# hobincar/reconstruction-network-for-video-captioning

Hardware: AMD Instinct MI355X
Metric: captions/sec (train step) MSVD bs=100 28x1536 feats (higher is better)
Workload: dtype bf16; 1 GPU; decoder + global reconstructor train step (fwd+bwd+clip+Adam), B=100 per GPU, F=28, D=R=1536, V=4188, E=468, H=512, A=128, T=31, dropout 0.5, LSTM cells; global_batch=100, parallelism=dp1, hipgraph=True, deferred_reconstructor_update=True, grad_allreduce=False

## Files before the change

### reconstruction-network-for-video-captioning_amd/csrc/abi_step.inc

```

int recnet_set_deferred_reconstructor_update(recnet_handle* h, int32_t on, void* stream) {
  REQUIRE_WS(h);
  FLUSH_PENDING(h, stream);
  h->defer_rec = on ? (on == 2 ? 2 : 1) : 0;
  LAUNCH_OK();
  return RECNET_OK;
}
int recnet_flush(recnet_handle* h, void* stream) {
  REQUIRE_WS(h);
  int r = flush_pending(h, (hipStream_t)stream, 1); if (r) return r;
  LAUNCH_OK();
  return RECNET_OK;
}
int recnet_set_dp_overlap(recnet_handle* h, int32_t on) {
  if (!h) return fail(RECNET_EINVAL, "null handle");
  h->dp_overlap = on ? 1 : 0;
  return RECNET_OK;
}
int recnet_join_side(recnet_handle* h, void* stream) {
  REQUIRE_WS(h);
  if (h->side_open && h->s2) { hipEventRecord(h->ev[14], h->s2); hipStreamWaitEvent((hipStream_t)stream, h->ev[14], 0); }
  h->side_open = 0;
  LAUNCH_OK();
  return RECNET_OK;
}
int recnet_abort_step(recnet_handle* h) {
  if (!h) return fail(RECNET_EINVAL, "null handle");
  h->dp_overlap = 0; h->side_open = 0; h->in_fused = 0; h->defer_now = 0; h->defer_err = 0;
  h->total_late = 0; h->side_tail_open = 0; h->rec_wait_pending = 0; h->rec_norm_late = 0; h->rec_loss_late = 0; h->rec_loss_defer = 0; h->prezeroed = 0; h->norms_hoisted = 0; h->hoist_pending = 0;
  h->hoist_fork_recorded = 0; h->side_fork_recorded = 0; h->encmean_hoisted = 0; h->ctx_done = 0; h->side_pending = 0;
  h->join_pending = 0; h->join_recorded = 0; h->deferred_done = 0; h->deferred_early = 0; h->early_opt_done = 0;
  h->xcat_done = 0; h->mp_done = 0; h->dhr_done = 0; h->dout_ready = 0; h->gg_slots = 0; h->gemm_single_group = 0;
  h->img_defer_now = 0; h->s3_late = 0;
  h->gws_cur = h->gws;
  return RECNET_OK;
}
int recnet_mark_pending(recnet_handle* h) {
  if (!h) return fail(RECNET_EINVAL, "null handle");
  if (h->defer_rec) { h->maybe_pending = 1; h->images_maybe_stale = 1; }
  return RECNET_OK;
}

int recnet_forward_decoder(recnet_handle* h, const float* enc, const int64_t* targets, int32_t T,
                           const float* step_weight, int32_t train, uint32_t seed, float* hiddens_out,
                           recnet_scalars* scalars, void* stream) {
  REQUIRE_WS(h);
  if (!h->dec_bound) return fail(RECNET_ESTATE, "decoder not bound");
  if (!enc || !targets || !step_weight) return fail(RECNET_EINVAL, "null argument");
  if (check_T(h, T)) return fail(RECNET_EINVAL, "T out of range");
  hipStream_t st = (hipStream_t)stream;
  hipLaunchKernelGGL(set_u32_kernel, dim3(1), dim3(1), 0, st, h->ctrl, seed);
  int r = fwd_decoder(h, enc, targets, T, step_weight, train, hiddens_out, st); if (r) return r;
  if (scalars) hipLaunchKernelGGL(export_scalars_kernel, dim3(1), dim3(1), 0, st, h->scal, scalars);
  LAUNCH_OK();
  return RECNET_OK;
}
// ... 150 lines not shown
    hipLaunchKernelGGL(mean_over_f_kernel, dim3(ew_blocks((size_t)h->B * h->D)), dim3(256), 0, sn, h->hoist_enc, h->B, h->F, h->D, h->encmean);
    h->encmean_hoisted = 1;
  }
  if (sn != st) hipEventRecord(h->ev[5], sd);
}

static void side_after_decoder_fwd(recnet_handle* h, hipStream_t st) {
  hipStream_t sd = h->overlap ? h->s2 : st;
  const bool par = sd != st;
  h->side_pending = 0;
  if (par) {
    if (h->side_fork_recorded) {
      hipStreamWaitEvent(sd, h->ev[0], 0);
      if (h->kind == RECNET_REC_GLOBAL && h->persist_rec) wait_chain(h, 2, sd);
    } else fork_to(h, 0, st, sd);
    h->side_fork_recorded = 0; h->gws_cur = h->gws2;
  }
  h->join_pending = par; h->join_recorded = 0; h->side_tail_open = 0;
  if (par && h->kind != RECNET_REC_NONE) h->gg_slots = 2 * (h->ncu > 192 ? h->ncu - 192 : 32);
  int r = dec_fwd_loss(h, h->side_targets, h->side_T, h->side_stepw, 1, sd);
  if (!r) r = dec_bwd_out(h, 1.0f, sd);
  h->gg_slots = 0;
  if (!r && par && h->side_phase != 2) { dec_ctx_rows(h, h->side_enc, 0, h->side_T, sd); h->ctx_done = 1; }
  if (h->side_tail_open) hipEventRecord(h->ev[18], sd);
  h->gws_cur = h->gws;
  h->side_err = r;
}

static int fwd_bwd_impl(recnet_handle* h, const float* enc, const int64_t* targets, int T, const float* stepw, hipStream_t st,
                        int phase, int early_opt) {
  const bool rec = h->kind != RECNET_REC_NONE;
  hipStream_t sd = h->overlap ? h->s2 : st;
  const bool par = sd != st;
  int r;
  bool s3_join = false;
  const float* dh = rec ? h->dHsrec : nullptr;
  h->early_opt_done = 0;
  if (phase != 2) h->free_fwd = 0;
  if (phase != 2) h->ctx_done = 0;
  const bool defer_static = h->defer_rec && (h->kind == RECNET_REC_GLOBAL || (h->defer_rec == 2 && h->kind == RECNET_REC_LOCAL)) && phase == 0 && early_opt >= 0 && par && h->s3 &&
                            (h->defer_rec != 2 || h->split_ok);
  const bool defer = defer_static && (h->defer_rec != 2 || T >= 2);
  if (!defer && h->defer_rec && phase != 2) {
    if (defer_static) { const int fr = flush_pending(h, st, 1); if (fr) return fr; }
    else if (h->maybe_pending) { const int fr = flush_pending(h, st, 0); if (fr) return fr; }
  }
// ... 110 lines not shown

int recnet_train_step_fwd_bwd(recnet_handle* h, const float* enc, const int64_t* targets, int32_t T,
                              const float* step_weight, uint32_t seed, recnet_scalars* scalars, void* stream) {
  REQUIRE_WS(h);
  FLUSH_PENDING(h, stream);
  if (!h->dec_bound || (h->kind != RECNET_REC_NONE && !h->rec_bound)) return fail(RECNET_ESTATE, "models not bound");
  if (!h->dGd.out_weight || (h->kind != RECNET_REC_NONE && !h->rG.out_weight)) return fail(RECNET_ESTATE, "gradients not bound");
  if (!enc || !targets || !step_weight) return fail(RECNET_EINVAL, "null argument");
  if (check_T(h, T)) return fail(RECNET_EINVAL, "T out of range");
  hipStream_t st = (hipStream_t)stream;
  hipLaunchKernelGGL(set_u32_kernel, dim3(1), dim3(1), 0, st, h->ctrl, seed);
  int r = fwd_bwd(h, enc, targets, T, step_weight, st); if (r) return r;
  if (scalars) hipLaunchKernelGGL(export_scalars_kernel, dim3(1), dim3(1), 0, st, h->scal, scalars);
  h->fwd_dec_done = 0;
  LAUNCH_OK();
  return RECNET_OK;
}

static void step_fail_cleanup(recnet_handle* h, hipStream_t st) {
  if (h->s3_late && h->s3) join_from(h, 11, st, h->s3);
  recnet_abort_step(h);
  if (h->defer_rec) { h->maybe_pending = 1; h->images_maybe_stale = 1; }
}
static int check_step_args(recnet_handle* h, const float* enc, const int64_t* targets, int T, const float* step_weight) {
  if (!h->dec_bound || (h->kind != RECNET_REC_NONE && !h->rec_bound)) return fail(RECNET_ESTATE, "models not bound");
  if (!h->dGd.out_weight || (h->kind != RECNET_REC_NONE && !h->rG.out_weight)) return fail(RECNET_ESTATE, "gradients not bound");
  if (!enc || !targets || !step_weight) return fail(RECNET_EINVAL, "null argument");
  if (check_T(h, T)) return fail(RECNET_EINVAL, "T out of range");
  return RECNET_OK;
}

int recnet_train_step(recnet_handle* h, const float* enc, const int64_t* targets, int32_t T,
                      const float* step_weight, uint32_t seed, int32_t step, recnet_scalars* scalars, void* stream) {
  REQUIRE_WS(h);
  if (!h->defer_rec) { const int fr_ = flush_pending(h, (hipStream_t)stream); if (fr_) return fr_; }
  int r = check_step_args(h, enc, targets, T, step_weight); if (r) return r;
  if (step < 1) return fail(RECNET_EINVAL, "step must be >= 1");
  hipStream_t st = (hipStream_t)stream;
  const int flags = RECNET_OPT_REG | RECNET_OPT_CLIP;
  hipLaunchKernelGGL(set_u32_kernel, dim3(1), dim3(1), 0, st, h->ctrl, seed);
  hipLaunchKernelGGL(set_step_kernel, dim3(1), dim3(1), 0, st, (int32_t*)(h->ctrl + 1), step);
  h->in_fused = 1;
  r = fwd_bwd(h, enc, targets, T, step_weight, st, 0, flags); if (r) { h->in_fused = 0; return r; }
  r = optimizer_step(h, flags, st, h->early_opt_done ? 0 : -1); h->in_fused = 0;
  if (r) { step_fail_cleanup(h, st); return r; }
  if (h->s3_late) { join_from(h, 11, st, h->s3); h->s3_late = 0; }
  h->img_defer_now = 0;
  if (scalars) hipLaunchKernelGGL(export_scalars_kernel, dim3(1), dim3(1), 0, st, h->scal, scalars);
  h->fwd_dec_done = 0;
  LAUNCH_OK();
  return RECNET_OK;
}

int recnet_train_step_dev(recnet_handle* h, const float* enc, const int64_t* targets, int32_t T, const float* step_weight,
                          uint32_t seed_base, int32_t flags, recnet_scalars* scalars, void* stream) {
  REQUIRE_WS(h);
  if (!h->defer_rec) { const int fr_ = flush_pending(h, (hipStream_t)stream); if (fr_) return fr_; }
  int r = check_step_args(h, enc, targets, T, step_weight); if (r) return r;
  hipStream_t st = (hipStream_t)stream;
  hipLaunchKernelGGL(advance_step_kernel, dim3(1), dim3(1), 0, st, (int32_t*)(h->ctrl + 1), h->ctrl, seed_base);
  h->in_fused = 1;
  r = fwd_bwd(h, enc, targets, T, step_weight, st, 0, flags); if (r) { h->in_fused = 0; return r; }
  r = optimizer_step(h, flags, st, h->early_opt_done ? 0 : -1); h->in_fused = 0;
  if (r) { step_fail_cleanup(h, st); return r; }
  if (h->s3_late) { join_from(h, 11, st, h->s3); h->s3_late = 0; }
  h->img_defer_now = 0;
  if (scalars) hipLaunchKernelGGL(export_scalars_kernel, dim3(1), dim3(1), 0, st, h->scal, scalars);
  h->fwd_dec_done = 0;
  LAUNCH_OK();
  return RECNET_OK;
}

int recnet_set_step(recnet_handle* h, int32_t step, void* stream) {
  REQUIRE_WS(h);
  hipLaunchKernelGGL(set_u32_kernel, dim3(1), dim3(1), 0, (hipStream_t)stream, h->ctrl + 1, (uint32_t)step);
  LAUNCH_OK();
  return RECNET_OK;
}

int recnet_train_step_fwd_bwd_dev(recnet_handle* h, const float* enc, const int64_t* targets, int32_t T,
                                  const float* step_weight, uint32_t seed_base, recnet_scalars* scalars, void* stream) {
  REQUIRE_WS(h);
  FLUSH_PENDING(h, stream);
  if (!h->dec_bound || (h->kind != RECNET_REC_NONE && !h->rec_bound)) return fail(RECNET_ESTATE, "models not bound");
  if (!h->dGd.out_weight || (h->kind != RECNET_REC_NONE && !h->rG.out_weight)) return fail(RECNET_ESTATE, "gradients not bound");
  if (!enc || !targets || !step_weight) return fail(RECNET_EINVAL, "null argument");
// ... 41 lines not shown
```

### reconstruction-network-for-video-captioning_amd/csrc/api.hip

```cpp
#include <hip/hip_runtime.h>
#include <math.h>
#include <stdio.h>
#include <stdlib.h>
#include <ctype.h>
#include <string.h>
#include <algorithm>
#include <string>
#include <vector>

#include "../../include/recnet_hip.h"
#include "kernels.hpp"
#include "rec_chain.hpp"
#include "dec_chain.hpp"
#include "loc_chain.hpp"
#include "loc_big.hpp"

static thread_local std::string g_err;
static int fail(int code, const std::string& m) { g_err = m; return code; }
#define HIPCHK(x) do { hipError_t e_ = (x); if (e_ != hipSuccess) return fail(RECNET_EHIP, std::string(#x) + ": " + hipGetErrorString(e_)); } while (0)
#define LAUNCH_OK() do { hipError_t e_ = hipGetLastError(); if (e_ != hipSuccess) return fail(RECNET_EHIP, std::string(__func__) + ": " + hipGetErrorString(e_)); } while (0)

static inline int cdiv(long a, long b) { return (int)((a + b - 1) / b); }
static inline int ew_blocks(size_t n) { size_t b = (n + 255) / 256; return (int)(b > 4096 ? 4096 : (b < 1 ? 1 : b)); }

struct OptGroup {
  std::vector<TensorDesc> tab;
  std::vector<int2> chunks;
  TensorDesc* d_tab = nullptr; int2* d_chunks = nullptr; PackDesc* d_pack = nullptr;
  std::vector<PackDesc> pack;
  float* d_partial = nullptr; float* d_pnorm = nullptr; float* d_gnorm = nullptr;
  int ntens = 0, nchunks = 0;
  bool bound = false;
};

static inline int pad8(int n) { return (n + 7) & ~7; }
#define RN_REC_T_WHH(h) ((h)->kind == RECNET_REC_LOCAL ? 5 : 1)
#define RN_GCNT_WORDS 16384
#define RN_MAX_ROW_GROUPS 4

struct recnet_handle {
  recnet_config c;
  int B, F, D, E, H, A, V, R, RA, Tm, kind, prec, cml;
  int dgru = 0, rgru = 0;
  int lp;
  int ldD, ldE, ldH, ldV, ldA, ld4H, ldWS, ldR, ld4R, ldRA, ldHR, ldRA4, ld2H;
  char* ws = nullptr; size_t ws_bytes = 0; size_t need = 0;
  uint32_t* ctrl;
  uint32_t* gbar;
  float* scal;
  float *slab2 = nullptr;
  float *bsum4 = nullptr, *bsum4r = nullptr;
  int prezeroed = 0;
  float *bsum_d, *Uv, *Xe, *Hs, *Cs, *acts, *Wh, *att, *logits, *rowloss, *slab, *gws, *dHs, *dHsrec, *dc_carry, *dUv,
      *dwacc, *demb, *stepw, *msep;
  void *enc_lp, *emb_lp, *Hs_lp, *P, *dlog_lp, *dGx, *ctx_lp, *dUv_lp, *dWhs;
  void *U_w, *Wc_w, *We_w, *Wcomb, *Wo_w;
  void* WcombT = nullptr;
  int ldKW = 0, use_wcomb_t = 0;
  float *bsum_r, *mp, *Xg, *Hr, *Cr, *acts_r, *hrmean, *outm, *encmean, *dhrmean, *dmpd, *dmp, *dcr_carry;
// ... 31 lines not shown
  int rec_norm_late = 0;
  int side_tail_open = 0;
  int total_late = 0;
  int split_ok = 0;
  int rec_wait_pending = 0;
  int defer_rec = 0, defer_now = 0, defer_err = 0, maybe_pending = 0, def_rows = 0, defer_flags = 3; hipStream_t s3 = nullptr; float* gws3 = nullptr;
  int mp_done = 0;
  int ncu = 0;
  int ctx_done = 0;
  int hoist_pending = 0, hoist_par = 0, encmean_hoisted = 0; const float* hoist_enc = nullptr;
  int xcat_done = 0;
  float* dc_G2 = nullptr; void* dc_pan2 = nullptr;
  void *Xcat_g, *Hr_lp, *hrmean_lp, *dout_lp, *dGr, *Xcat_r, *dUd_lp, *dWhr, *dWhrs, *Wr4_w;
  void *Wih_f, *Whh_w, *Wor_w, *Ur_w, *Wr_w, *Wihh_w;
  int persist_rec = 0;
  float *sr_logits, *sr_scores, *sr_h[2], *sr_c[2], *sr_hn, *sr_cn, *sr_cum[2], *sr_vals;
  int64_t *sr_tok[2], *sr_hist[2]; int32_t *sr_eos[2], *sr_idx;
  int64_t* in_tok = nullptr;
  int free_fwd = 0;
  size_t gws_floats, slab_floats;
  float* gws2 = nullptr; float* gws_cur = nullptr;
  unsigned* gcnt = nullptr;
  int gg_site = 0;
  struct RnSw { int wait_chain = 1, mse_epi = 1, adam_epi = 1, dec_lw = 1, dec_xcat = 1, rec_epi = 2, rec_wide = 1, persist_ms = 0, gemm_group = 1; } sw;
  int gg_slots = 0;
  int gemm_single_group = 0;
  hipStream_t s2 = nullptr; hipEvent_t ev[24] = {}; int overlap = 1;
  recnet_decoder_tensors dP{}, dGd{}, dM{}, dV{}, dVm{};
  recnet_reconstructor_tensors rP{}, rG{}, rM{}, rV{}, rVm{};
  bool dec_bound = false, rec_bound = false;
  OptGroup og[2];
  int T_last = 0, train_last = 0, fwd_dec_done = 0, fwd_rec_done = 0, rec_bwd_done = 0, early_opt_done = 0, norms_hoisted = 0, join_pending = 0;
  int prof_on = 0; std::vector<hipEvent_t> prof_ev; size_t prof_used = 0;
};

static size_t carve(recnet_handle* h, char* base) {
  size_t off = 0;
  auto take = [&](size_t nfloats) -> float* {
    float* p = base ? (float*)(base + off) : nullptr;
    off += ((nfloats * 4 + 255) / 256) * 256;
    return p;
  };
  auto takev = [&](size_t n) -> void* { return (void*)take(n); };
  const size_t B = h->B, F = h->F, D = h->D, E = h->E, H = h->H, A = h->A, V = h->V, R = h->R, RA = h->RA, Tm = h->Tm;
  h->ldD = pad8(h->D); h->ldE = pad8(h->E); h->ldH = pad8(h->H); h->ldV = pad8(h->V); h->ldA = pad8(h->A);
  h->ld4H = pad8(4 * h->H); h->ldWS = pad8(4 * h->H + RN_FCH * h->A);
  h->ldR = pad8(h->R); h->ld4R = pad8(4 * h->R); h->ldRA = pad8(h->RA); h->ldHR = pad8(h->H + h->R);
// ... 101 lines not shown
      if (h->lc_steps) h->Wst = takev((R / 16) * 4 * (size_t)(h->lc_steps - h->lc_sr) * 4 * 512 / 2 + 64);
    }
    h->lc_pang = takev(F * rc_pan_elems((int)(4 * R)) / 2 + 64);
    h->lc_panw = takev(F * rc_pan_elems((int)RA) / 2 + 64);
    h->lc_dx = take(F * 4 * B * H);
    h->WihhT = takev((H + R) * (size_t)h->ld4R);
    if (R > 2048 && R % 128 == 0 && B <= 64 * 2 * RN_MAX_ROW_GROUPS) {
      const int steps = (int)R / 128;
      h->lb_steps = steps; h->lb_sr = LB_SR(steps); h->lb_ncb = (int)(H + R) / 64;
      h->lb_part = take(F * 4 * 64 * (H + R));
      h->lb_dxm = take(F * B * H); h->lb_dbeta = take(F * B * Tm);
      h->WstT = takev((size_t)h->lb_ncb * 4 * 4 * (size_t)(steps - h->lb_sr) * 4 * 512 / 2 + 64);
    }
  }
  for (int g = 0; g < 2; ++g) {
    OptGroup& o = h->og[g];
    size_t nparams = g == 0 ? (V * E + A * H + A * D + 2 * A + 4 * H * (E + D) + 4 * H * H + 8 * H + V * H + V)
                            : (RA * R + RA * H + 2 * RA + 4 * R * 2 * H + 4 * R * R + 8 * R + R * R + R);
    size_t maxch = nparams / RN_CHUNK + 16;
    o.d_tab = (TensorDesc*)take(16 * sizeof(TensorDesc) / 4);
    o.d_pack = (PackDesc*)take(16 * sizeof(PackDesc) / 4);
    o.d_chunks = (int2*)take(maxch * 2);
    o.d_partial = take(maxch);
    o.d_pnorm = take(16);
    o.d_gnorm = take(16);
  }
  return off;
}

static DropDesc mkdrop(const recnet_handle* h, uint32_t site, float p, int train) {
  DropDesc d;
  d.seed = h->ctrl; d.site = site;
  d.thr = train ? rn_drop_thr(p) : 0u;
  d.inv_keep = (p < 1.f) ? 1.0f / (1.0f - p) : 0.f;
  d.Bg = h->c.global_batch_size; d.boff = h->c.batch_offset;
  return d;
}

extern "C" {

int recnet_abi_version(void) { return RECNET_ABI_VERSION; }
const char* recnet_last_error(void) { return g_err.c_str(); }

static std::vector<std::string> env_list(const char* var) {
  std::vector<std::string> out;
  const char* e = getenv(var);
// ... 13 lines not shown
int recnet_create(const recnet_config* cfg, recnet_handle** out) {
  if (!cfg || !out) return fail(RECNET_EINVAL, "null argument");
  const recnet_config& c = *cfg;
  if (c.batch_size <= 0 || c.encoder_output_len <= 0 || c.encoder_output_size <= 0 || c.embedding_size <= 0 ||
      c.decoder_hidden_size <= 0 || c.decoder_attn_size <= 0 || c.n_vocabs <= 3 || c.caption_max_len <= 0)
    return fail(RECNET_EINVAL, "non-positive dimension");
  if (c.reconstructor_type < 0 || c.reconstructor_type > 2) return fail(RECNET_EINVAL, "unknown reconstructor_type");
  if (c.precision != RECNET_PREC_F32 && c.precision != RECNET_PREC_BF16) return fail(RECNET_EINVAL, "unknown precision");
  if (c.decoder_attn_normalize != RECNET_ATTN_NONE && c.decoder_attn_normalize != RECNET_ATTN_SOFTMAX)
    return fail(RECNET_EINVAL, "unknown decoder_attn_normalize (0 = none, 1 = softmax)");
  if (c.decoder_cell < 0 || c.decoder_cell > 1 || c.reconstructor_cell < 0 || c.reconstructor_cell > 1)
    return fail(RECNET_EINVAL, "unknown recurrent cell (0 = LSTM, 1 = GRU)");
  if (c.reconstructor_type != RECNET_REC_NONE && c.reconstructor_hidden_size <= 0)
    return fail(RECNET_EINVAL, "reconstructor_hidden_size");
  if (c.reconstructor_type == RECNET_REC_LOCAL && c.reconstructor_hidden_size != c.encoder_output_size)
    return fail(RECNET_EINVAL, "local reconstructor requires reconstructor_hidden_size == encoder_output_size (train.py:128)");
  if (c.reconstructor_type == RECNET_REC_GLOBAL && c.reconstructor_hidden_size != c.encoder_output_size)
    return fail(RECNET_EINVAL, "global reconstructor requires reconstructor_hidden_size == encoder_output_size (train.py:101)");
  if (c.reconstructor_type == RECNET_REC_LOCAL && c.reconstructor_attn_size <= 0)
    return fail(RECNET_EINVAL, "reconstructor_attn_size");
  const std::vector<std::string> per_step = env_list("RN_PER_STEP"), alts = env_list("RN_ALT");
  const std::vector<std::string> per_step_names = {"dec", "dec_bwd", "rec", "rec_bwd", "loc", "loc_bwd", "loc_big", "all"};
  const std::vector<std::string> alt_names = {"dec_wh_in_phase_a", "dec_no_xcat", "rec_epilogue_0", "rec_epilogue_1", "rec_bwd_narrow",
                                              "rec_row_parts_1", "rec_row_parts_2", "loc_no_hybrid", "loc_xsplit_never", "loc_xsplit_always"};
  for (const std::string& t : per_step) if (!has(per_step_names, t)) return fail(RECNET_EINVAL, "RN_PER_STEP: unknown name '" + t + "'");
  for (const std::string& t : alts) if (!has(alt_names, t)) return fail(RECNET_EINVAL, "RN_ALT: unknown name '" + t + "'");
  auto alt = [&](const char* name) { return has(alts, name); };
  auto chain_on = [&](const char* name) { return !has(per_step, name) && !has(per_step, "all"); };
  recnet_handle* h = new recnet_handle();
  h->c = c;
  if (h->c.global_batch_size <= 0) h->c.global_batch_size = c.batch_size;
  h->B = c.batch_size; h->F = c.encoder_output_len; h->D = c.encoder_output_size; h->E = c.embedding_size;
  h->H = c.decoder_hidden_size; h->A = c.decoder_attn_size; h->V = c.n_vocabs;
  h->R = c.reconstructor_type ? c.reconstructor_hidden_size : 0;
  h->RA = c.reconstructor_type == RECNET_REC_LOCAL ? c.reconstructor_attn_size : 0;
  h->cml = c.caption_max_len; h->Tm = c.caption_max_len + 1;
  h->kind = c.reconstructor_type; h->prec = c.precision; h->lp = c.precision == RECNET_PREC_BF16;
  h->gemm_single_group = 0;
  {
    auto env = [](const char* n, int dflt) { const char* e = getenv(n); return e ? atoi(e) : dflt; };
    h->sw.wait_chain = env("RN_WAIT_CHAIN", 1); h->sw.mse_epi = env("RN_MSE_EPILOGUE", 1); h->sw.adam_epi = env("RN_ADAM_EPILOGUE", 1);
    h->sw.gemm_group = env("RN_GEMM_GROUP", 1);
    h->sw.dec_lw = !alt("dec_wh_in_phase_a");
    h->sw.dec_xcat = !alt("dec_no_xcat"); h->sw.rec_epi = alt("rec_epilogue_0") ? 0 : (alt("rec_epilogue_1") ? 1 : 2); h->sw.rec_wide = !alt("rec_bwd_narrow");
    h->sw.persist_ms = alt("rec_row_parts_1") ? 1 : (alt("rec_row_parts_2") ? 2 : 0);
  }
  h->dgru = c.decoder_cell == RECNET_CELL_GRU; h->rgru = c.reconstructor_type != RECNET_REC_NONE && c.reconstructor_cell == RECNET_CELL_GRU;
  {
    const char* eg = getenv("RN_ROW_GROUPS");
    int ng = (h->B + RC_PAN_ROWS - 1) / RC_PAN_ROWS;
    if (eg && atoi(eg) == 0 && ng > 1) ng = 0;
    h->bgrp = ng >= 1 && ng <= RN_MAX_ROW_GROUPS ? (h->B + ng - 1) / ng : h->B;
  }
  const int Bg = h->bgrp;
  {
    int dev = 0, ncu = 0;
    hipGetDevice(&dev);
    hipDeviceGetAttribute(&ncu, hipDeviceAttributeMultiprocessorCount, dev);
    h->ncu = ncu;
    h->persist_rec = chain_on("rec") && h->lp && h->kind == RECNET_REC_GLOBAL && Bg <= RC_PAN_ROWS && h->Tm <= 60 &&
                     (h->R & 7) == 0 && h->R <= 2048 && h->R / 8 <= ncu;
    const int N = 4 * h->H + h->A, NA = N / 16;
    h->persist_dec = chain_on("dec") && h->lp && h->Tm <= 60 && (h->H & 7) == 0 && h->H <= 512 && h->F <= 32 + DC_XF && h->A <= 128 &&
                     (N & 15) == 0 && Bg <= RC_PAN_ROWS && (NA > Bg ? NA : Bg) + 1 <= ncu;
    h->persist_rec_bwd = chain_on("rec_bwd") && h->persist_rec && (h->R & 15) == 0;
  }
  h->bgrp_loc = h->bgrp;
  {
// ... 252 lines not shown
```

### reconstruction-network-for-video-captioning_amd/csrc/host_reconstructor.inc

```
static void lstm_pw(recnet_handle* h, int Hd, int S, int slab_ld, const float* X, int x_ld, const float* b1, const float* b2,
                    const float* c_prev, float* h_out, void* h_lp, int hlp_ld, void* h_lp2, int hlp2_ld, float* c_out,
                    float* acts, hipStream_t st) {
  LstmPwArgs p;
  p.B = h->B; p.Hd = Hd; p.S = S; p.gru = h->rgru; p.slab = h->slab; p.slab_stride = (size_t)h->B * slab_ld; p.slab_ld = slab_ld;
  p.X = X; p.x_ld = x_ld; p.b1 = b1; p.b2 = b2; p.c_prev = c_prev; p.h_out = h_out; p.h_ld = Hd;
  p.h_lp = h_lp; p.hlp_ld = hlp_ld; p.hlp_pad_from = Hd; p.h_lp2 = h_lp2; p.hlp2_ld = hlp2_ld; p.c_out = c_out; p.acts = acts;
  auto al16 = [](const void* q) { return (((uintptr_t)q) & 15) == 0; };
  const bool vec = (Hd & 3) == 0 && (slab_ld & 3) == 0 && (x_ld & 3) == 0 && (hlp_ld & 3) == 0 && (hlp2_ld & 3) == 0 &&
                   al16(p.slab) && al16(X) && al16(b1) && al16(b2) && al16(c_prev) && al16(h_out) && al16(c_out) && al16(acts) &&
                   (((uintptr_t)h_lp) & 7) == 0 && (((uintptr_t)h_lp2) & 7) == 0;
  if (vec) LAUNCH_AT(h, lstm_pw_vec_kernel, dim3(cdiv((long)h->B * (Hd >> 2), 256)), dim3(256), 0, st, p);
  else LAUNCH_AT(h, lstm_pw_kernel, dim3(cdiv((long)h->B * Hd, 256)), dim3(256), 0, st, p);
}
static void mean_over_t(recnet_handle* h, const float* X, int T, int Cn, float scale, float* out, void* out_lp, int ld_lp, hipStream_t st) {
  const size_t n = (size_t)h->B * (out_lp ? ld_lp : Cn);
  if (h->lp) hipLaunchKernelGGL(mean_over_t_kernel<bf16_t>, dim3(ew_blocks(n)), dim3(256), 0, st, X, T, h->B, Cn, scale, out, (bf16_t*)out_lp, ld_lp);
  else hipLaunchKernelGGL(mean_over_t_kernel<float>, dim3(ew_blocks(n)), dim3(256), 0, st, X, T, h->B, Cn, scale, out, (float*)out_lp, ld_lp);
}

template <typename K, typename Args>
static void rc_launch(recnet_handle* h, int site, K kern, dim3 grid, size_t smem, hipStream_t st, const Args& a) {
  if (smem > 64 * 1024) hipFuncSetAttribute(reinterpret_cast<const void*>(kern), hipFuncAttributeMaxDynamicSharedMemorySize, (int)smem);
  hipEvent_t e1 = nullptr;
  if (h->prof_on == site) {
// ... 573 lines not shown
    }
    e.ad_pnorm = o.d_pnorm + ti;
  };
  if (!h->rgru) add(0, 4 * R, 0, dG1);
  else { add(0, 2 * R, 0, dG1); add((size_t)2 * R, R, (size_t)3 * R, at_off(h, (void*)dG1, (size_t)3 * R)); }
  h->gg_site = 3;
  if (!gg_run(h, g, s, &sh)) return false;
  if (local) { refresh_wst(h, s); refresh_wihh_t(h, s, 2); }
  return true;
}
static int optimizer_step(recnet_handle* h, int flags, hipStream_t st, int only_group, int deferred, int step_off, unsigned skip_mask) {
  RN_RANGE("recnet: norms + clip + Adam (train.py:270-273)");
  for (int g = 0; g < 2; ++g) {
    OptGroup& o = h->og[g];
    if (!o.bound) continue;
    if (only_group >= 0 && g != only_group) continue;
    if (g == 0 && (flags & RECNET_OPT_SKIP_DECODER)) continue;
    if (g == 1 && ((flags & RECNET_OPT_SKIP_RECONSTRUCTOR) || h->kind == RECNET_REC_NONE)) continue;
    if (!o.tab[0].m || !o.tab[0].g) return fail(RECNET_ESTATE, "gradients / Adam state not bound");
    AdamHyper hp = adam_hyper(h, g, flags);
    const float coef = hp.reg_coef;
    const float* clip = nullptr;
    if (g == 0 && (flags & RECNET_OPT_CLIP) && h->c.gradient_clip > 0.f) {
      hipLaunchKernelGGL(sumsq_chunk_kernel, dim3(o.nchunks), dim3(256), 0, st, o.d_tab, o.d_chunks, 1, o.d_pnorm, coef, o.d_partial);
      if (o.ntens <= 16) {
        hipLaunchKernelGGL(norm_all_kernel, dim3(1), dim3(256), 0, st, o.d_tab, o.d_partial, o.ntens, o.d_gnorm, h->c.gradient_clip, h->scal + 7, h->scal + 8, (float*)nullptr);
      } else {
        hipLaunchKernelGGL(tensor_norm_kernel, dim3(o.ntens), dim3(256), 0, st, o.d_tab, o.d_partial, o.d_gnorm);
        hipLaunchKernelGGL(norm_finalize_kernel, dim3(1), dim3(64), 0, st, o.d_gnorm, o.ntens, h->c.gradient_clip, h->scal + 7, h->scal + 8, (float*)nullptr);
      }
      clip = h->scal + 8;
    }
    hipLaunchKernelGGL(adam_chunk_kernel, dim3(o.nchunks), dim3(256), 0, st, o.d_tab, o.d_chunks, hp, o.d_pnorm, clip,
                       (const int32_t*)(h->ctrl + 1), (const PackDesc*)o.d_pack, h->lp, (const float*)(h->scal + 15),
                       deferred ? (const uint32_t*)(h->ctrl + 2) : (const uint32_t*)nullptr, step_off, g == 1 ? skip_mask : 0u);
    if (g == 0) refresh_wcomb_t(h, st);
    if (g == 1) rec_images_after_update(h, st, (skip_mask >> RN_REC_T_WHH(h)) & 1u);
  }
  return RECNET_OK;
}
```

### reconstruction-network-for-video-captioning_amd/csrc/loc_chain.hpp

```cpp
#pragma once
#include "common.hpp"
#include "rec_chain.hpp"

struct LocChainArgs {
  int F, T, B, R, H, A, gru;
  int Bs;
  int NU, NG, MS, NC;
  int relay;
  const bf16_t* W; int ldw;
  const bf16_t* Wr; int ldwr;
  const bf16_t* Wst;
  const float* bias;
  const float* Hs; const float* Ud;
  const float* ab; const float* w;
  float* Hr; float* Cr; float* acts;
  bf16_t* Hlp; int ld_hlp;
  bf16_t* Xcat; int ld_xcat;
  float* beta; float* Whr;
  bf16_t* PanH; bf16_t* PanX;
  _Float16* Pw;
  unsigned* bar; unsigned* epoch; float* poison;
  DropDesc dd;
  unsigned long long* ts;
};
// ... 32 lines not shown
  if (threadIdx.x < 64) {
    const unsigned* r = rel + (blockIdx.x & 7) * 32;
    unsigned spin = 0;
    while ((int)(__hip_atomic_load(r, __ATOMIC_RELAXED, __HIP_MEMORY_SCOPE_AGENT) - target) < 0) { if (rc_give_up(bar, spin)) break; }
    if (RC_ACQUIRE_INV) __builtin_amdgcn_fence(__ATOMIC_ACQUIRE, "agent");
  }
  __syncthreads();
}
__device__ __forceinline__ void lc_wait_or_relay(bool me, unsigned* rel, const unsigned* flags, int n, unsigned target, unsigned* bar) {
  if (!me) { lc_wait(rel, target, bar); return; }
  if (threadIdx.x < 64) {
    unsigned spin = 0;
    lc_poll(flags, n, target, bar, spin);
    lc_release(rel, target);
    if (RC_ACQUIRE_INV) __builtin_amdgcn_fence(__ATOMIC_ACQUIRE, "agent");
  }
  __syncthreads();
}
__device__ __forceinline__ void lc_arrive(unsigned* flag, unsigned v) {
  if (threadIdx.x == 0) __hip_atomic_store(flag, v, __ATOMIC_RELAXED, __HIP_MEMORY_SCOPE_AGENT);
}
__device__ __forceinline__ void lc_store16f(float* dst, f32x4 v) { rc_store16f(dst, v); }
__device__ __forceinline__ void lc_store16(bf16_t* dst, const bf16_t* src) { rc_store16(dst, src); }
#define LC_GLOBAL __attribute__((address_space(1)))
typedef const LC_GLOBAL bf16x8* lc_gbf16x8;
typedef const LC_GLOBAL f32x4* lc_gf32x4;
typedef const LC_GLOBAL float* lc_gf32;
template <typename T> __device__ __forceinline__ const LC_GLOBAL T* lc_launder_v(const T* ptr) { asm volatile("" : "+v"(ptr)); return (const LC_GLOBAL T*)ptr; }
template <typename T> __device__ __forceinline__ const LC_GLOBAL T* lc_launder_s(const T* ptr) { asm volatile("" : "+s"(ptr)); return (const LC_GLOBAL T*)ptr; }
typedef short lc_s4 __attribute__((ext_vector_type(4)));
typedef _Float16 lc_h4 __attribute__((ext_vector_type(4)));

template <int STEPS, int PF, int RB, int SR = STEPS, int NQ = 32>
__global__ __launch_bounds__(256) void loc_chain_kernel(const LocChainArgs p) {
  constexpr int CG = 4, UW = 16, ROWS = RB * 16, NP = STEPS / 2, KG = UW / 8, SX = 4, NPR = SR / 2;
  static_assert(SR % 2 == 0 && SR <= STEPS && SR >= 2 * PF, "resident k-steps: whole pairs, at least the prefetch distance");
  extern __shared__ __attribute__((aligned(16))) float lc_smem[];
  const int tid = threadIdx.x, lane = tid & 63, wave = __builtin_amdgcn_readfirstlane(tid >> 6);
  const int wg = blockIdx.x, R = p.R, B = p.B, Bs = p.Bs, H = p.H, A = p.A, F = p.F, T = p.T;
  const unsigned ep = rc_epoch_read(p.epoch), fb = ep << 7;
  unsigned* relU = p.bar + 256; unsigned* relC = p.bar + 256 + 16;
  const size_t pan_h = rc_pan_elems(R), pan_x = rc_pan_elems(H);

  if (p.relay && wg == p.NU + p.NC) {
    if (tid < 64) {
      unsigned spin = 0;
// ... 169 lines not shown
  }
  constexpr int CPT = (ROWS * UW + 255) / 256;
  static_assert(CPT == 4 || CPT == 2, "RB = 4 or 2");
#define LCU_CELL(c) (((tid / UW) * CPT + (c)) * UW + tid % UW)
  float xb[CPT][4], cpv[CPT];
  bool mine[CPT];
#pragma unroll
  for (int c = 0; c < CPT; ++c) {
    const int cell = LCU_CELL(c), rg = r0 + cell / UW;
    mine[c] = cell < ROWS * UW && rg >= own_lo && rg < own_lo + own && rg < B;
    cpv[c] = 0.f;
#pragma unroll
    for (int q = 0; q < 4; ++q) xb[c][q] = p.bias[q * R + u0 + cell % UW];
  }
  const int lane_off = ((lane >> 4) * RC_PAN_ROWS + r0 + (lane & 15)) * 8;
  f32x4 acc[RB][CG];
#pragma unroll
  for (int i = 0; i < RB; ++i)
#pragma unroll
    for (int g = 0; g < CG; ++g) acc[i][g] = f32x4{0.f, 0.f, 0.f, 0.f};
  const int it_j = tid / own, it_rg = own_lo + tid % own;
  const bool it_on = tid < KG * own && it_rg < B && it_rg - r0 < ROWS;
  const bf16_t* it_src = hl + (it_on ? it_rg - r0 : 0) * UW + (it_on ? it_j : 0) * 8;

  for (int s = 0; s < F; ++s) {
    lc_wait(relC, fb + (unsigned)(s + 1), p.bar);
    if (wg == 0) LC_TS(0, s, 0);
    {
      const bf16_t* Ax = p.PanX + (size_t)s * pan_x + lane_off;
      bf16x8 fx[SX][RB];
#pragma unroll
      for (int ks = 0; ks < SX; ++ks) {
        const int k = (wave * SX + ks) * 32;
#pragma unroll
        for (int i = 0; i < RB; ++i) fx[ks][i] = *reinterpret_cast<const bf16x8*>(Ax + ((k < H ? (k >> 3) : 0) * RC_PAN_ROWS + i * 16) * 8);
      }
#pragma unroll
      for (int ks = 0; ks < SX; ++ks)
#pragma unroll
        for (int g = 0; g < CG; ++g) {
          const bf16x8 bw = wih[((wave * SX + ks) * CG + g) * 64 + lane];
#pragma unroll
          for (int i = 0; i < RB; ++i) acc[i][g] = __builtin_amdgcn_mfma_f32_16x16x32_bf16(fx[ks][i], bw, acc[i][g], 0, 0, 0);
        }
    }
    {
// ... 28 lines not shown
        }
      }
    }
    float hv[CPT], av[CPT][4];
#pragma unroll
    for (int c = 0; c < CPT; ++c) {
      const int cell = LCU_CELL(c);
      float g4[4];
#pragma unroll
      for (int q = 0; q < 4; ++q) g4[q] = xb[c][q] + gsum[q][c];
      if (p.gru) {
        const GruOut r = gru_point(g4[0], g4[1], g4[2], g4[3], cpv[c]);
        hv[c] = r.h; av[c][0] = r.r; av[c][1] = r.z; av[c][2] = r.n; av[c][3] = r.hn; cpv[c] = r.h;
      } else {
        const LstmOut r = lstm_point(g4[0], g4[1], g4[2], g4[3], cpv[c]);
        hv[c] = r.h; av[c][0] = r.i; av[c][1] = r.f; av[c][2] = r.g; av[c][3] = r.o; cpv[c] = r.c;
      }
      if (cell < ROWS * UW) hl[cell] = (bf16_t)hv[c];
    }
    __syncthreads();
    if (wg == 0) LC_TS(0, s, 2);
    const bool more = s + 1 < F;
    if (more) {
      if (it_on) lc_store16(p.PanH + (size_t)s * pan_h + ((size_t)(ug * KG + it_j) * RC_PAN_ROWS + it_rg) * 8, it_src);
      {
        _Float16* Pn = p.Pw + ((size_t)(s + 1) * B * p.NG + ug) * A;
#pragma unroll
        for (int i = 0; i < RB; ++i) {
          const bf16x4 fa = *reinterpret_cast<const bf16x4*>(hl + (i * 16 + (lane & 15)) * UW + (lane >> 4) * 4);
          const int rg = r0 + i * 16 + (lane & 15);
          const bool ron = rg >= own_lo && rg < own_lo + own && rg < B;
#pragma unroll
          for (int q = 0; q < 2; ++q) {
            const int a0 = (2 * wave + q) * 16 + (lane >> 4) * 4;
            if ((2 * wave + q) * 16 < A) {
              const f32x4 d = __builtin_amdgcn_mfma_f32_16x16x16bf16_1k(__builtin_bit_cast(lc_s4, wr[q]), __builtin_bit_cast(lc_s4, fa),
                                                                        f32x4{0.f, 0.f, 0.f, 0.f}, 0, 0, 0);
              if (ron && a0 < A) {
                union { lc_h4 h; uint64_t u; } pk;
                pk.h[0] = (_Float16)d[0]; pk.h[1] = (_Float16)d[1]; pk.h[2] = (_Float16)d[2]; pk.h[3] = (_Float16)d[3];
                __hip_atomic_store(reinterpret_cast<uint64_t*>(Pn + (size_t)rg * p.NG * A + a0), pk.u, __ATOMIC_RELAXED, __HIP_MEMORY_SCOPE_AGENT);
              }
            }
          }
        }
      }
      if (wg == 0) LC_TS(0, s, 3);
      asm volatile("s_waitcnt vmcnt(0)" ::: "memory");
      __syncthreads();
      lc_arrive(p.bar + wg, fb + (unsigned)(s + 1));
      if (wg == 0) LC_TS(0, s, 4);
    }
    float* Ht = p.Hr + (size_t)s * Bs * R;
    float* Ct = p.Cr + (size_t)s * Bs * R;
    float* At = p.acts + (size_t)s * Bs * 4 * R;
    bf16_t* Lt = p.Hlp + (size_t)s * Bs * p.ld_hlp;
    if (it_on) *reinterpret_cast<bf16x8*>(Lt + (size_t)it_rg * p.ld_hlp + u0 + it_j * 8) = *reinterpret_cast<const bf16x8*>(it_src);
#pragma unroll
    for (int c = 0; c < CPT; ++c) {
      const int cell = LCU_CELL(c);
      if (mine[c]) {
        const int row = r0 + cell / UW, u = u0 + cell % UW;
        const size_t o = (size_t)row * R + u;
        Ht[o] = hv[c];
        if (!p.gru) Ct[o] = cpv[c];
        float* a = At + (size_t)row * 4 * R + u;
        a[0] = av[c][0]; a[R] = av[c][1]; a[2 * R] = av[c][2]; a[3 * R] = av[c][3];
      }
    }
    if (wg == 0 && p.ld_hlp > R)
      for (int jj = tid; jj < B * (p.ld_hlp - R); jj += 256) Lt[(size_t)(jj / (p.ld_hlp - R)) * p.ld_hlp + R + jj % (p.ld_hlp - R)] = (bf16_t)0.f;
    if (more) {
      bf16x8 fw[PF][2][CG];
      const LC_GLOBAL bf16_t* wsl = (const LC_GLOBAL bf16_t*)wst;
      if constexpr (SR < STEPS) wsl = lc_launder_v(wst);
      auto issue_w = [&](int slot, int i) {
#pragma unroll
        for (int hh = 0; hh < 2; ++hh)
#pragma unroll
          for (int g = 0; g < CG; ++g) fw[slot][hh][g] = *(lc_gbf16x8)(wsl + (size_t)(((i * 2 + hh) * CG + g) * 512));
      };
      constexpr int NPS = NP - NPR;
      auto pair_of = [&](int i) { return i < NPS ? NPR + i : i - NPS; };
      if constexpr (NPS > 0) {
#pragma unroll
        for (int i = 0; i < PF; ++i)
          if (i < NPS) issue_w(i % PF, i);
      }
      lc_wait(relU, fb + (unsigned)(s + 1), p.bar);
// ... 560 lines not shown
```

Before: 68600 captions/s.

## Overlap decoder output-weight gradient norm with side stream; narrow loc_chain addressing

Before the optimizer step, the sum-of-squares partials for the decoder's output-weight and trailing tensor chunks are now computed on the side stream right after the decoder backward. The optimizer's clip pass then only reduces the remaining chunks into a separate partial buffer, shortening the serial tail. The local-chain kernel also precomputes 32-bit offsets and uses an inline-asm global store for the panel write to cut address arithmetic. Risks include ordering between the side-stream norm and later gradient writes, and 32-bit offset overflow; the local-chain change does not run for the global reconstructor.

Result: no change. 68230 captions/s (-0.5%).

```diff
diff --git a/reconstruction-network-for-video-captioning_amd/csrc/abi_step.inc b/reconstruction-network-for-video-captioning_amd/csrc/abi_step.inc
--- a/reconstruction-network-for-video-captioning_amd/csrc/abi_step.inc
+++ b/reconstruction-network-for-video-captioning_amd/csrc/abi_step.inc
@@ -31,7 +31,7 @@
   h->hoist_fork_recorded = 0; h->side_fork_recorded = 0; h->encmean_hoisted = 0; h->ctx_done = 0; h->side_pending = 0;
   h->join_pending = 0; h->join_recorded = 0; h->deferred_done = 0; h->deferred_early = 0; h->early_opt_done = 0;
   h->xcat_done = 0; h->mp_done = 0; h->dhr_done = 0; h->dout_ready = 0; h->gg_slots = 0; h->gemm_single_group = 0;
-  h->img_defer_now = 0; h->s3_late = 0;
+  h->img_defer_now = 0; h->s3_late = 0; h->early_norm = 0; h->early_norm_done = 0;
   h->gws_cur = h->gws;
   return RECNET_OK;
 }
@@ -228,6 +228,12 @@
   if (!r) r = dec_bwd_out(h, 1.0f, sd);
   h->gg_slots = 0;
   if (!r && par && h->side_phase != 2) { dec_ctx_rows(h, h->side_enc, 0, h->side_T, sd); h->ctx_done = 1; }
+  if (!r && h->early_norm) {
+    OptGroup& o = h->og[0];
+    const int c0 = o.tab[RN_DEC_T_OUTW].chunk0;
+    hipLaunchKernelGGL(sumsq_chunk_kernel, dim3(o.nchunks - c0), dim3(256), 0, sd, o.d_tab, o.d_chunks + c0, 1, o.d_pnorm, h->early_norm_coef, o.d_gpart + c0);
+    h->early_norm_done = 1;
+  }
   if (h->side_tail_open) hipEventRecord(h->ev[18], sd);
   h->gws_cur = h->gws;
   h->side_err = r;
@@ -384,6 +390,13 @@
   recnet_abort_step(h);
   if (h->defer_rec) { h->maybe_pending = 1; h->images_maybe_stale = 1; }
 }
+static void early_norm_begin(recnet_handle* h, int flags) {
+  const OptGroup& o = h->og[0];
+  h->early_norm_done = 0;
+  h->early_norm = !h->sw.tail_sumsq && (flags & RECNET_OPT_CLIP) && !(flags & RECNET_OPT_SKIP_DECODER) && h->c.gradient_clip > 0.f &&
+                  o.bound && o.ntens == RN_DEC_T_OUTW + 2 && o.tab[0].g && o.tab[0].m;
+  h->early_norm_coef = adam_hyper(h, 0, flags).reg_coef;
+}
 static int check_step_args(recnet_handle* h, const float* enc, const int64_t* targets, int T, const float* step_weight) {
   if (!h->dec_bound || (h->kind != RECNET_REC_NONE && !h->rec_bound)) return fail(RECNET_ESTATE, "models not bound");
   if (!h->dGd.out_weight || (h->kind != RECNET_REC_NONE && !h->rG.out_weight)) return fail(RECNET_ESTATE, "gradients not bound");
@@ -402,9 +415,9 @@
   const int flags = RECNET_OPT_REG | RECNET_OPT_CLIP;
   hipLaunchKernelGGL(set_u32_kernel, dim3(1), dim3(1), 0, st, h->ctrl, seed);
   hipLaunchKernelGGL(set_step_kernel, dim3(1), dim3(1), 0, st, (int32_t*)(h->ctrl + 1), step);
-  h->in_fused = 1;
-  r = fwd_bwd(h, enc, targets, T, step_weight, st, 0, flags); if (r) { h->in_fused = 0; return r; }
-  r = optimizer_step(h, flags, st, h->early_opt_done ? 0 : -1); h->in_fused = 0;
+  h->in_fused = 1; early_norm_begin(h, flags);
+  r = fwd_bwd(h, enc, targets, T, step_weight, st, 0, flags); h->early_norm = 0; if (r) { h->in_fused = 0; h->early_norm_done = 0; return r; }
+  r = optimizer_step(h, flags, st, h->early_opt_done ? 0 : -1); h->in_fused = 0; h->early_norm_done = 0;
   if (r) { step_fail_cleanup(h, st); return r; }
   if (h->s3_late) { join_from(h, 11, st, h->s3); h->s3_late = 0; }
   h->img_defer_now = 0;
@@ -421,9 +434,9 @@
   int r = check_step_args(h, enc, targets, T, step_weight); if (r) return r;
   hipStream_t st = (hipStream_t)stream;
   hipLaunchKernelGGL(advance_step_kernel, dim3(1), dim3(1), 0, st, (int32_t*)(h->ctrl + 1), h->ctrl, seed_base);
-  h->in_fused = 1;
-  r = fwd_bwd(h, enc, targets, T, step_weight, st, 0, flags); if (r) { h->in_fused = 0; return r; }
-  r = optimizer_step(h, flags, st, h->early_opt_done ? 0 : -1); h->in_fused = 0;
+  h->in_fused = 1; early_norm_begin(h, flags);
+  r = fwd_bwd(h, enc, targets, T, step_weight, st, 0, flags); h->early_norm = 0; if (r) { h->in_fused = 0; h->early_norm_done = 0; return r; }
+  r = optimizer_step(h, flags, st, h->early_opt_done ? 0 : -1); h->in_fused = 0; h->early_norm_done = 0;
   if (r) { step_fail_cleanup(h, st); return r; }
   if (h->s3_late) { join_from(h, 11, st, h->s3); h->s3_late = 0; }
   h->img_defer_now = 0;
diff --git a/reconstruction-network-for-video-captioning_amd/csrc/api.hip b/reconstruction-network-for-video-captioning_amd/csrc/api.hip
--- a/reconstruction-network-for-video-captioning_amd/csrc/api.hip
+++ b/reconstruction-network-for-video-captioning_amd/csrc/api.hip
@@ -29,12 +29,14 @@
   TensorDesc* d_tab = nullptr; int2* d_chunks = nullptr; PackDesc* d_pack = nullptr;
   std::vector<PackDesc> pack;
   float* d_partial = nullptr; float* d_pnorm = nullptr; float* d_gnorm = nullptr;
+  float* d_gpart = nullptr;
   int ntens = 0, nchunks = 0;
   bool bound = false;
 };
 
 static inline int pad8(int n) { return (n + 7) & ~7; }
 #define RN_REC_T_WHH(h) ((h)->kind == RECNET_REC_LOCAL ? 5 : 1)
+#define RN_DEC_T_OUTW 9
 #define RN_GCNT_WORDS 16384
 #define RN_MAX_ROW_GROUPS 4
 
@@ -112,7 +114,8 @@
   float* gws2 = nullptr; float* gws_cur = nullptr;
   unsigned* gcnt = nullptr;
   int gg_site = 0;
-  struct RnSw { int wait_chain = 1, mse_epi = 1, adam_epi = 1, dec_lw = 1, dec_xcat = 1, rec_epi = 2, rec_wide = 1, persist_ms = 0, gemm_group = 1; } sw;
+  struct RnSw { int wait_chain = 1, mse_epi = 1, adam_epi = 1, dec_lw = 1, dec_xcat = 1, rec_epi = 2, rec_wide = 1, persist_ms = 0, gemm_group = 1, tail_sumsq = 0; } sw;
+  int early_norm = 0, early_norm_done = 0; float early_norm_coef = 0.f;
   int gg_slots = 0;
   int gemm_single_group = 0;
   hipStream_t s2 = nullptr; hipEvent_t ev[24] = {}; int overlap = 1;
@@ -260,6 +263,7 @@
     o.d_pack = (PackDesc*)take(16 * sizeof(PackDesc) / 4);
     o.d_chunks = (int2*)take(maxch * 2);
     o.d_partial = take(maxch);
+    o.d_gpart = take(maxch);
     o.d_pnorm = take(16);
     o.d_gnorm = take(16);
   }
@@ -319,7 +323,7 @@
   const std::vector<std::string> per_step = env_list("RN_PER_STEP"), alts = env_list("RN_ALT");
   const std::vector<std::string> per_step_names = {"dec", "dec_bwd", "rec", "rec_bwd", "loc", "loc_bwd", "loc_big", "all"};
   const std::vector<std::string> alt_names = {"dec_wh_in_phase_a", "dec_no_xcat", "rec_epilogue_0", "rec_epilogue_1", "rec_bwd_narrow",
-                                              "rec_row_parts_1", "rec_row_parts_2", "loc_no_hybrid", "loc_xsplit_never", "loc_xsplit_always"};
+                                              "rec_row_parts_1", "rec_row_parts_2", "loc_no_hybrid", "loc_xsplit_never", "loc_xsplit_always", "tail_sumsq_pass"};
   for (const std::string& t : per_step) if (!has(per_step_names, t)) return fail(RECNET_EINVAL, "RN_PER_STEP: unknown name '" + t + "'");
   for (const std::string& t : alts) if (!has(alt_names, t)) return fail(RECNET_EINVAL, "RN_ALT: unknown name '" + t + "'");
   auto alt = [&](const char* name) { return has(alts, name); };
@@ -341,6 +345,7 @@
     h->sw.dec_lw = !alt("dec_wh_in_phase_a");
     h->sw.dec_xcat = !alt("dec_no_xcat"); h->sw.rec_epi = alt("rec_epilogue_0") ? 0 : (alt("rec_epilogue_1") ? 1 : 2); h->sw.rec_wide = !alt("rec_bwd_narrow");
     h->sw.persist_ms = alt("rec_row_parts_1") ? 1 : (alt("rec_row_parts_2") ? 2 : 0);
+    h->sw.tail_sumsq = alt("tail_sumsq_pass");
   }
   h->dgru = c.decoder_cell == RECNET_CELL_GRU; h->rgru = c.reconstructor_type != RECNET_REC_NONE && c.reconstructor_cell == RECNET_CELL_GRU;
   {
diff --git a/reconstruction-network-for-video-captioning_amd/csrc/host_reconstructor.inc b/reconstruction-network-for-video-captioning_amd/csrc/host_reconstructor.inc
--- a/reconstruction-network-for-video-captioning_amd/csrc/host_reconstructor.inc
+++ b/reconstruction-network-for-video-captioning_amd/csrc/host_reconstructor.inc
@@ -619,11 +619,15 @@
     const float coef = hp.reg_coef;
     const float* clip = nullptr;
     if (g == 0 && (flags & RECNET_OPT_CLIP) && h->c.gradient_clip > 0.f) {
-      hipLaunchKernelGGL(sumsq_chunk_kernel, dim3(o.nchunks), dim3(256), 0, st, o.d_tab, o.d_chunks, 1, o.d_pnorm, coef, o.d_partial);
+      const bool early = h->early_norm_done && h->early_norm_coef == coef && o.ntens == RN_DEC_T_OUTW + 2;
+      h->early_norm_done = 0;
+      const int nlate = early ? o.tab[RN_DEC_T_OUTW].chunk0 : o.nchunks;
+      float* const part = early ? o.d_gpart : o.d_partial;
+      hipLaunchKernelGGL(sumsq_chunk_kernel, dim3(nlate), dim3(256), 0, st, o.d_tab, o.d_chunks, 1, o.d_pnorm, coef, part);
       if (o.ntens <= 16) {
-        hipLaunchKernelGGL(norm_all_kernel, dim3(1), dim3(256), 0, st, o.d_tab, o.d_partial, o.ntens, o.d_gnorm, h->c.gradient_clip, h->scal + 7, h->scal + 8, (float*)nullptr);
+        hipLaunchKernelGGL(norm_all_kernel, dim3(1), dim3(256), 0, st, o.d_tab, part, o.ntens, o.d_gnorm, h->c.gradient_clip, h->scal + 7, h->scal + 8, (float*)nullptr);
       } else {
-        hipLaunchKernelGGL(tensor_norm_kernel, dim3(o.ntens), dim3(256), 0, st, o.d_tab, o.d_partial, o.d_gnorm);
+        hipLaunchKernelGGL(tensor_norm_kernel, dim3(o.ntens), dim3(256), 0, st, o.d_tab, part, o.d_gnorm);
         hipLaunchKernelGGL(norm_finalize_kernel, dim3(1), dim3(64), 0, st, o.d_gnorm, o.ntens, h->c.gradient_clip, h->scal + 7, h->scal + 8, (float*)nullptr);
       }
       clip = h->scal + 8;
diff --git a/reconstruction-network-for-video-captioning_amd/csrc/loc_chain.hpp b/reconstruction-network-for-video-captioning_amd/csrc/loc_chain.hpp
--- a/reconstruction-network-for-video-captioning_amd/csrc/loc_chain.hpp
+++ b/reconstruction-network-for-video-captioning_amd/csrc/loc_chain.hpp
@@ -78,6 +78,10 @@
 }
 __device__ __forceinline__ void lc_store16f(float* dst, f32x4 v) { rc_store16f(dst, v); }
 __device__ __forceinline__ void lc_store16(bf16_t* dst, const bf16_t* src) { rc_store16(dst, src); }
+__device__ __forceinline__ void lc_store16_at(const bf16_t* base, unsigned byte_off, const bf16_t* src) {
+  const f32x4 v = *reinterpret_cast<const f32x4*>(src);
+  asm volatile("global_store_dwordx4 %0, %1, %2 sc1\n\ts_nop 1" :: "v"(byte_off), "v"(v), "s"(base) : "memory");
+}
 #define LC_GLOBAL __attribute__((address_space(1)))
 typedef const LC_GLOBAL bf16x8* lc_gbf16x8;
 typedef const LC_GLOBAL f32x4* lc_gf32x4;
@@ -293,6 +297,8 @@
   const int it_j = tid / own, it_rg = own_lo + tid % own;
   const bool it_on = tid < KG * own && it_rg < B && it_rg - r0 < ROWS;
   const bf16_t* it_src = hl + (it_on ? it_rg - r0 : 0) * UW + (it_on ? it_j : 0) * 8;
+  const unsigned it_lo = it_on ? (unsigned)(it_rg * p.ld_hlp + u0 + it_j * 8) : 0u;
+  const unsigned it_off = it_on ? (unsigned)(((ug * KG + it_j) * RC_PAN_ROWS + it_rg) * 8) * 2u : 0u;
 
   for (int s = 0; s < F; ++s) {
     lc_wait(relC, fb + (unsigned)(s + 1), p.bar);
@@ -367,7 +373,7 @@
     if (wg == 0) LC_TS(0, s, 2);
     const bool more = s + 1 < F;
     if (more) {
-      if (it_on) lc_store16(p.PanH + (size_t)s * pan_h + ((size_t)(ug * KG + it_j) * RC_PAN_ROWS + it_rg) * 8, it_src);
+      if (it_on) lc_store16_at(p.PanH + (size_t)s * pan_h, it_off, it_src);
       {
         _Float16* Pn = p.Pw + ((size_t)(s + 1) * B * p.NG + ug) * A;
 #pragma unroll
@@ -400,16 +406,16 @@
     float* Ct = p.Cr + (size_t)s * Bs * R;
     float* At = p.acts + (size_t)s * Bs * 4 * R;
     bf16_t* Lt = p.Hlp + (size_t)s * Bs * p.ld_hlp;
-    if (it_on) *reinterpret_cast<bf16x8*>(Lt + (size_t)it_rg * p.ld_hlp + u0 + it_j * 8) = *reinterpret_cast<const bf16x8*>(it_src);
+    if (it_on) *reinterpret_cast<bf16x8*>(Lt + it_lo) = *reinterpret_cast<const bf16x8*>(it_src);
 #pragma unroll
     for (int c = 0; c < CPT; ++c) {
       const int cell = LCU_CELL(c);
       if (mine[c]) {
         const int row = r0 + cell / UW, u = u0 + cell % UW;
-        const size_t o = (size_t)row * R + u;
+        const unsigned o = (unsigned)(row * R + u);
         Ht[o] = hv[c];
         if (!p.gru) Ct[o] = cpv[c];
-        float* a = At + (size_t)row * 4 * R + u;
+        float* a = At + (unsigned)(row * 4 * R + u);
         a[0] = av[c][0]; a[R] = av[c][1]; a[2 * R] = av[c][2]; a[3 * R] = av[c][3];
       }
     }
```
